# Sabre94/k8s-llm-monitor

Measured on AMD Instinct MI355X. Metric: diagnostic queries/sec (Llama-3-8B TP=1, /api/v1/query), higher is better.
Workload: dtype bf16; 1 GPU; model=llama-3-8b, global_batch=64, seq_len=2263, max_model_len=8192, parallelism=tp1, mode=wave, client=process, weight_layout=one (fragment-packed)

## Files before the change

k8s_llm_monitor_amd/ops/__init__.py:

```python
from __future__ import annotations

import importlib
import math
from collections import OrderedDict
from typing import Optional

import torch

from . import cpu_attn
from . import reference as ref

_EXT = None
_EXT_ERR: Optional[BaseException] = None


def native():
    global _EXT, _EXT_ERR
    if _EXT is None and _EXT_ERR is None:
        try:
            _EXT = importlib.import_module("k8s_llm_monitor_amd.ops._k8sllm_ops")
        except BaseException as e:
            _EXT_ERR = e
    if _EXT is None:
        raise RuntimeError(
# ... 438 lines not shown
    F2, K = w13.shape
    F = F2 // 2
    if F % 8:
        raise ValueError("interleave_gate_up8: F must be a multiple of 8")
    return w13.reshape(2, F // 8, 8, K).permute(1, 0, 2, 3).reshape(F2, K)


def deinterleave_gate_up8(w: torch.Tensor) -> torch.Tensor:
    F2, K = w.shape
    return w.reshape(F2 // 16, 2, 8, K).permute(1, 0, 2, 3).reshape(F2, K)


DEC_TABLE: dict = {
    (6144, 4096, 0): (4, 1, 6, 8),
    (4096, 4096, 0): (8, 1, 8, 8),
    (28672, 4096, 2): (1, 1, 7, 8),
    (4096, 14336, 0): (8, 1, 8, 8),
    (128256, 4096, 1): (1, 4, 8, 4),
    (151936, 4096, 1): (1, 2, 8, 8),
}

DEC_TABLE_M128: dict = {
    (6144, 4096, 0): (4, 1, 6, 8),
    (4096, 4096, 0): (8, 1, 8, 8),
    (28672, 4096, 2): (1, 1, 7, 8),
    (4096, 14336, 0): (8, 1, 8, 8),
    (128256, 4096, 1): (1, 2, 8, 8),
}


DEC_TABLE_F8: dict = {}

DEC_TABLE_F4: dict = {}


def dec_config(N: int, K: int, epi: int, experts: int = 1, rows: int = 0, f8: bool = False,
               f4: bool = False) -> Optional[tuple]:
    if (f8 or f4) and experts != 1:
        return None
    return _dec_pick(N, K, epi, experts, rows, f8, f4)


def _dec_pick(N: int, K: int, epi: int, experts: int, rows: int, f8: bool, f4: bool) -> Optional[tuple]:
    wide = rows > DEC_NARROW_MAX_M
    if wide and (experts != 1 or rows > DEC_MAX_M):
        return None
    if f8 and K % 64:
        return None
    if f4 and (f8 or K % 128):
        return None
    compiled = ([DEC_FORMS[i] for i in DEC_F8_FORMS] if f8 else
                [DEC_FORMS[i] for i, _ in DEC_F4_FORMS] if f4 else DEC_FORMS)
    if f8 and experts == 1 and (N, K, epi, 128 if wide else 64) in DEC_TABLE_F8:
        return DEC_TABLE_F8[(N, K, epi, 128 if wide else 64)]
    if f4 and experts == 1 and (N, K, epi, 128 if wide else 64) in DEC_TABLE_F4:
        return DEC_TABLE_F4[(N, K, epi, 128 if wide else 64)]
    hit = (DEC_TABLE_M128 if wide else DEC_TABLE).get((N, K, epi)) if experts == 1 else None
    if hit is not None and (not f8 or dec_form_ok(epi, hit, rows, f8=True)) and (
            not f4 or dec_form_ok(epi, hit, rows, f4=True, K=K)):
        return hit
    ntiles, ksteps = N // 16, K // 32
    forms = [f[1:4] for f in compiled
             if f[0] == epi and rows <= 16 * f[4] and f[:4] not in DEC_FORMS_TABLE_ONLY]
    cands = [(s,) + f for s in ((1, 2, 4, 8, 16) if epi == DEC_SLAB else (1,)) for f in forms]
    best = None
    for s, ntw, w, d in cands:
# ... 90 lines not shown
        for e in range(max(E, 1)):
            x = _cpu_a(a[e] if a.dim() == 5 else a, rows).float()
            wf = _cpu_w(w[e], wscale[e] if enc else None) if E else _cpu_w(w, wscale)
            if epi == 0:
                kc = K // S
                slabs = workspace[e * S * M * N: (e + 1) * S * M * N].view(S, M, N)
                for s in range(S):
                    y = x[:, s * kc:(s + 1) * kc] @ wf[:, s * kc:(s + 1) * kc].t()
                    slabs[s] = y * sc if sc is not None else y
                if row_w is not None:
                    slabs.mul_(row_w[:M, e].float().view(1, M, 1))
                continue
            y = x @ wf.t()
            if sc is not None:
                y = y * sc
            o = out[e] if E else out
            if epi == 1:
                o[:M].copy_(y.to(o.dtype))
            else:
                gu = deinterleave_gate_up8(y.to(a.dtype).float().t()).t()
                g, u = gu[:, : N // 2], gu[:, N // 2:]
                o.copy_(pack_activation((torch.nn.functional.silu(g) * u).to(a.dtype)))
        return max(E, 1) * S if epi == 0 else 1
    rn = (None, 0.0) if rownorm is None else (rownorm[0], float(rownorm[1]))
    wn = rownorm is not None and rownorm[0].shape[1] > 16
    ok = (dec_grouped_q_form_ok(epi, cfg, M, K=K, **enc_kw(w)) if E and enc else
          dec_form_ok(epi, cfg, M, grouped=E > 0, wide_norm=wn, f8=f8, f4=f4, K=K))
    if not ok:
        raise RuntimeError(f"{name}: form (epi, ntw, waves, depth) = {(epi,) + tuple(cfg[1:])} not compiled for "
                           f"{M} rows" + (" of a grouped launch" if E else "") +
                           (" with the wide deferred norm" if wn else "") +
                           (" over fp8 weights" if f8 else f" over mxfp4 weights in {S} K slices" if f4 else ""))
    r = native().gemm_dec(a, w, wscale if enc else None, workspace, out, S, epi, ntw, waves, depth, M, *rn,
                          row_w if E else None, DEC_F4_DEPTH_FORCE if f4 else 0)
    if r < 0:
        raise RuntimeError(f"{name}: configuration {cfg} not compiled for N={N} K={K} epi={epi}")
    return r


def dec_gemm(a: torch.Tensor, wp: torch.Tensor, epi: int, rows: int, workspace: Optional[torch.Tensor] = None,
             out: Optional[torch.Tensor] = None, rownorm: Optional[tuple] = None,
             cfg: Optional[tuple] = None, wscale: Optional[torch.Tensor] = None) -> int:
    return _dec_gemm("gemm_dec", a, wp, wscale, epi, rows, workspace, out, rownorm, None, cfg, 0)


def dec_gemm_grouped(a: torch.Tensor, wp: torch.Tensor, epi: int, rows: int, workspace: Optional[torch.Tensor] = None,
                     out: Optional[torch.Tensor] = None, row_w: Optional[torch.Tensor] = None,
                     cfg: Optional[tuple] = None) -> int:
    if wp.dtype == torch.uint8:
        raise ValueError("gemm_dec_grouped: grouped launches have no mxfp4 form here (dec_gemm_grouped_q takes the "
                         "codes with their scales)")
    return _dec_gemm("gemm_dec_grouped", a, wp, None, epi, rows, workspace, out, None, row_w, cfg, wp.shape[0])


def dec_gemm_grouped_q(a: torch.Tensor, wq: torch.Tensor, wqs: torch.Tensor, epi: int, rows: int,
                       workspace: Optional[torch.Tensor] = None, out: Optional[torch.Tensor] = None,
                       row_w: Optional[torch.Tensor] = None, cfg: Optional[tuple] = None) -> int:
    E = grouped_q_wdims(wq)[0]
    return _dec_gemm("gemm_dec_grouped_q", a, wq, wqs, epi, rows, workspace, out, None, row_w, cfg, E)


def dec_gemm_rc(a: torch.Tensor, wp: torch.Tensor, rows: int, residual: torch.Tensor, norm_w: torch.Tensor,
                eps: float) -> Optional[tuple]:
    N, K = skinny_wdims(wp)
    M = rows
    if K % 256 or N % 32 or M > 64:
        return None
# ... 929 lines not shown
```

k8s_llm_monitor_amd/ops/csrc/bindings.cpp:

```cpp
#include <torch/extension.h>
#include <c10/hip/HIPStream.h>
#include <hip/hip_runtime.h>

#include <cmath>

#include "gemm_dec_forms.h"
#include "gemm_skinny_plan.h"
#include "gemm_tile_forms.h"
#include "paged_decode_forms.h"

extern "C" {
int k8sllm_rmsnorm(void* out, const void* x, void* residual, const void* w, long rows, int d, float eps,
                   long x_stride, long out_stride, hipStream_t s);
int k8sllm_layernorm(void* out, const void* x, const void* w, const void* b, long rows, int d, float eps,
                     hipStream_t s);
int k8sllm_silu_mul(void* out, const void* x, long rows, int F, int interleaved, hipStream_t s);
int k8sllm_gelu_tanh(void* out, const void* x, long n, hipStream_t s);
int k8sllm_embedding(void* out, const int* ids, const void* weight, long T, int d, int vocab_start, int rows,
                     hipStream_t s);
int k8sllm_resolve_ids(int* out, const int* ids, const int* src, const int* prev, int n, hipStream_t s);
int k8sllm_rope_cache(void* qkv, long qkv_stride, const int* positions, const float* cos_sin, void* k_cache,
                      void* v_cache, const int* slot_mapping, long T, int Hq, int Hkv, int D, int block_size,
                      int apply_rope, const float* partial, int S, float* kv_scale, const void* q_norm_w,
                      const void* k_norm_w, float eps, int norm_bf16, hipStream_t s);
// ... 22 lines not shown
                            int nrows, const int* tok_off, const void* blob, int V, const int* eos_ids, int n_eos,
                            hipStream_t s);
int k8sllm_penalty_reset(void* table, long tstride, int V, int nslots, int slot, const int* ids, int n_prompt,
                         int n_out, float* pparams, float rep, float inv_rep, float presence, float frequency,
                         hipStream_t s);
int k8sllm_sample_parts(long B, int V);
long k8sllm_token_logprobs_ws(long B, int V);
int k8sllm_token_logprobs(int* out, const void* logits, int is_fp32, long B, long stride, int V, const int* tok,
                          const int* want, void* ws, hipStream_t s);
int k8sllm_moe_route(const void* logits, long T, int E, int K, int renorm, int* topk_ids, float* topk_w,
                     hipStream_t s);
int k8sllm_moe_router(const void* x, const void* wr, long T, int d, int E, int K, int renorm, int* ids, float* w,
                      float* wd, hipStream_t s);
int k8sllm_moe_align(const int* topk_ids, long n, int E, int* expert_offsets, int* sorted_idx, int* inv_idx,
                     hipStream_t s);
int k8sllm_moe_combine(void* out, const void* expert_out, const int* inv_idx, const float* topk_w, long T, int K,
                       int d, hipStream_t s);
int k8sllm_gather_rows(void* out, const void* x, const int* idx, long n, int d, int div, hipStream_t s);
int k8sllm_gemm_tile(const void* X, const void* W, void* Y, int M, int N, int K, const int* offsets, int E, long w_es,
                     int epi, int algo, const int* rope_pos, const float* rope_cs, int rope_heads,
                     const float* rs_part, int rs_np, float rs_eps, void* resid, void* hw, const void* norm_w,
                     float* ss_out, int wpk, const void* wscale, int wfmt, int persist, int cus, hipStream_t s);
int k8sllm_gemm_tile_forms(int* out, int cap);
int k8sllm_gemm_tile_persist_forms(int* out, int cap);
int k8sllm_moe_grouped_gemm(const void* X, const void* W, void* Y, const int* offsets, int E, long rows, int N, int K,
                            long w_es, int epi, hipStream_t s);
int k8sllm_gemm_skinny(const void* A, long lda, const void* Wp, float* partial, void* Y, long ldy, int M, int N, int K,
                       int S, int epi, int nt_tiles, int a_packed, const float* rn_ss, int rn_nc, int rn_d,
                       float rn_eps, int waves, int experts, long w_es, long a_es, long y_es,
                       const float* row_w, int row_w_ld, int w_rm, hipStream_t s);
int k8sllm_gemm_dec(const void* A, const void* W, const void* wscale, int wf, float* partial, void* Y, long ldy, int M,
                    int N, int K, int splits, int epi, int ntw, int waves, int depth, int f4_depth, const float* rn_ss,
                    int rn_nc, int rn_d, float rn_eps, int experts, long a_es, long w_eb, long s_eb, long y_es,
                    const float* rw, int rw_ld, hipStream_t s);
int k8sllm_gemm_dec_forms(int* out, int cap);
int k8sllm_gemm_dec_f8_forms(int* out, int cap);
int k8sllm_gemm_dec_f4_forms(int* out, int cap);
int k8sllm_gemm_dec_rc(const void* A, const void* Wp, void* resid, const void* nw, void* xw, float* ss, int M, int N,
                       int K, hipStream_t s);
int k8sllm_add_norm_partial(void* out, long out_stride, void* residual, const float* partial, int S, int M,
                            const void* w, int d, float* ss_part, hipStream_t s);
int k8sllm_embed_norm_partial(void* out, long out_stride, void* residual, const int* ids, const int* src,
                              const int* prev, const void* emb, int vocab, const void* w, int M, int d,
                              float* ss_part, hipStream_t s);
int k8sllm_reduce_slabs(void* out, const float* partial, int S, long n, hipStream_t s);
int k8sllm_reduce_add_rmsnorm(void* out, void* residual, const float* partial, int S, int M, const void* w, int d,
                              float eps, long out_stride, void* out2, hipStream_t s);
void* k8sllm_car_create(int rank, int world, long max_elems, void* handles, int* err);
int k8sllm_car_handle_size();
int k8sllm_car_open(void* state, const void* all_handles);
int k8sllm_car_all_reduce(void* state, const void* in, void* out, long n, long spin_limit, int algo, hipStream_t s);
int k8sllm_car_fused_tail(void* state, const float* slabs, int ns, long slab_stride, void* residual, const void* w,
                          void* out, long ldo, int M, int d, float eps, int packed, long spin_limit, int algo,
                          hipStream_t s);
int k8sllm_car_error(void* state);
int k8sllm_car_all_gather(void* state, const void* in, void* out, long n, long spin_limit, hipStream_t s);
int k8sllm_car_all_to_all(void* state, const void* in, void* out, long n, long spin_limit, hipStream_t s);
int k8sllm_car_error_async(void* state, void* host_dst, hipStream_t s);
void k8sllm_car_destroy(void* state);
}

namespace {

hipStream_t cur() { return c10::hip::getCurrentHIPStream().stream(); }

void check(int rc, const char* what) { TORCH_CHECK(rc == 0, "k8sllm kernel launch failed: ", what, " rc=", rc); }

// ... 677 lines not shown
  } else {
    TORCH_CHECK(a.dim() == 2 && a.stride(1) == 1 && a.stride(0) % 8 == 0, "gemm_skinny: a layout");
    TORCH_CHECK(a.size(1) == K, "gemm_skinny: a has ", a.size(1), " columns, weight K=", K);
    M = (int)a.size(0);
  }
  const int S = epi == 0 ? (int)splits : 1;
  const auto p = k8sllm::skinny_plan(M, N, K, S, (int)epi, (int)nt_tiles, a_packed ? 1 : 0, (int)waves, 1, w_rm);
  TORCH_CHECK(p.err == 0, "gemm_skinny: at most ", k8sllm::kSkinnyMaxM, " rows of a shape it tiles, rc=", p.err);
  float* pp = nullptr;
  void* yp = nullptr;
  long ldy = 0;
  if (epi == 0) {
    pp = slab_buffer(partial, (int64_t)p.slabs * M * N, "gemm_skinny");
  } else if (epi == 3) {
    yp = swiglu_packed_out(y, 0, M, N, "gemm_skinny");
  } else {
    TORCH_CHECK(y.has_value(), "gemm_skinny: output tensor required");
    dev_bf16(*y, "y");
    const int ncol = epi == 2 ? N / 2 : N;
    TORCH_CHECK(y->dim() == 2 && y->size(0) >= M && y->size(1) == ncol && y->stride(1) == 1, "gemm_skinny: y shape");
    ldy = y->stride(0);
    yp = y->data_ptr();
  }
  const float* rp = nullptr;
  int rn_nc = 0;
  rownorm_args(rn_ss, M, K, rp, rn_nc);
  check(k8sllm_gemm_skinny(a.data_ptr(), a_packed ? 0 : a.stride(0), wp.data_ptr(), pp, yp, ldy, M, N, K, S, (int)epi,
                           (int)nt_tiles, a_packed ? 1 : 0, rp, rn_nc, K, (float)rn_eps, (int)waves, 1, 0, 0, 0,
                           nullptr, 0, w_rm, cur()),
        "gemm_skinny");
  return p.slabs;
}

int64_t gemm_dec(torch::Tensor a, torch::Tensor w, c10::optional<torch::Tensor> wscale,
                 c10::optional<torch::Tensor> partial, c10::optional<torch::Tensor> y, int64_t splits, int64_t epi,
                 int64_t ntw, int64_t waves, int64_t depth, int64_t rows, c10::optional<torch::Tensor> rn_ss,
                 double rn_eps, c10::optional<torch::Tensor> row_w, int64_t f4_depth) {
  dev_bf16(a, "a");
  const auto wt = w.scalar_type();
  const int wf = wt == torch::kFloat8_e4m3fn ? k8sllm::DEC_W_F8 : wt == torch::kUInt8 ? k8sllm::DEC_W_F4 : k8sllm::DEC_W_BF16;
  const int g = w.dim() == 5 ? 1 : 0;
  const int kq = wf == k8sllm::DEC_W_F4 ? 128 : wf == k8sllm::DEC_W_F8 ? 64 : 32, wl = wf == k8sllm::DEC_W_BF16 ? 8 : 16;
  const std::string whats = std::string("gemm_dec (") + (wf == k8sllm::DEC_W_F4 ? "mxfp4" : wf == k8sllm::DEC_W_F8 ? "fp8" : "bf16") +
                            (g ? ", grouped)" : ")");
  const char* what = whats.c_str();
  TORCH_CHECK(w.is_cuda() && (wf != k8sllm::DEC_W_BF16 || wt == torch::kBFloat16) && w.dim() == 4 + g &&
                  w.is_contiguous() && w.size(g + 2) == 64 && w.size(g + 3) == wl,
              what, ": w must be bf16 [N/16, K/32, 64, 8], float8_e4m3fn [N/16, K/64, 64, 16] or uint8 [N/16, K/128, "
                    "64, 16], fragment-packed, or an [E, ...] stack of such");
  const int E = g ? (int)w.size(0) : 0, N = (int)w.size(g) * 16, K = (int)w.size(g + 1) * kq, M = (int)rows;
  const void* sp = nullptr;
  if (wf == k8sllm::DEC_W_F8) {
    TORCH_CHECK(wscale.has_value() && wscale->is_cuda() && wscale->scalar_type() == torch::kFloat32 &&
                    wscale->is_contiguous() && (g ? wscale->dim() == 2 && wscale->size(0) == E && wscale->size(1) == N
                                                  : wscale->numel() == N),
                what, ": wscale must be [N] fp32 ([E, N] for a stack)");
    sp = wscale->data_ptr();
  } else if (wf == k8sllm::DEC_W_F4) {
    TORCH_CHECK(wscale.has_value() && wscale->is_cuda() && wscale->scalar_type() == torch::kUInt8 &&
                    wscale->is_contiguous() && wscale->dim() == 4 + g && (!g || wscale->size(0) == E) &&
                    wscale->size(g) == w.size(g) && wscale->size(g + 1) == w.size(g + 1) &&
                    wscale->size(g + 2) == 16 && wscale->size(g + 3) == 4,
                what, ": wscale must be uint8 [N/16, K/128, 16, 4] ([E, ...] for a stack)");
    sp = wscale->data_ptr();
  }
  TORCH_CHECK(g || !row_w.has_value(), what, ": routing weights go with an [E, ...] stack");
  TORCH_CHECK(!g || !rn_ss.has_value(), what, ": a grouped launch takes no deferred norm");
  TORCH_CHECK(!g || epi == 0 || epi == 2, what, ": only the slab and SwiGLU outputs");
  const float* rp = nullptr;
  int rn_nc = 0;
  rownorm_args(rn_ss, M, K, rp, rn_nc);
  const bool scaled = epi == 0 && row_w.has_value();
  const k8sllm::DecPlan p = k8sllm::dec_plan(wf, M, N, K, (int)splits, (int)epi, (int)ntw, (int)waves, (int)depth,
                                             (int)f4_depth, E, scaled, rn_nc);
  const int MT = (M + 15) / 16;
  TORCH_CHECK(M > 0 && M <= p.max_m && (!g || E >= 1), what, ": 1..", p.max_m, " rows", g ? ", >= 1 expert" : "");
  const bool per_e = g && a.dim() == 5;
  const int ag = per_e ? 1 : 0;
  TORCH_CHECK(a.is_contiguous() && a.dim() == 4 + ag && (!per_e || a.size(0) == E) && a.size(ag) >= MT &&
                  a.size(ag + 1) * 32 == K && a.size(ag + 2) == 64 && a.size(ag + 3) == 8,
              what, ": a must be fragment-packed [ceil(M/16), K/32, 64, 8]", g ? " or [E, ...]" : "");
  if (p.err < 0) return -1;
  float* pp = nullptr;
  void* yp = nullptr;
  long ldy = 0, y_es = 0;
  const float* rw = nullptr;
  int rw_ld = 0;
  if (epi == 0) {
    pp = slab_buffer(partial, (int64_t)p.slabs * M * N, what);
    if (scaled) {
      TORCH_CHECK(row_w->is_cuda() && row_w->scalar_type() == torch::kFloat32 && row_w->dim() == 2 &&
                      row_w->size(0) >= M && row_w->size(1) == E && row_w->stride(1) == 1,
                  what, ": row_w [M, E] fp32");
      rw = row_w->data_ptr<float>();
      rw_ld = (int)row_w->stride(0);
    }
  } else if (epi == 2) {
    yp = swiglu_packed_out(y, E, M, N, what);
    y_es = g ? y->stride(0) : 0;
  } else {
    TORCH_CHECK(y.has_value(), what, ": output tensor required");
    dev_bf16(*y, "y");
    TORCH_CHECK(y->dim() == 2 && y->size(0) >= M && y->size(1) == N && y->stride(1) == 1, what, ": y [M, N]");
    ldy = y->stride(0);
    yp = y->data_ptr();
  }
  const long a_es = per_e ? a.stride(0) : 0, w_eb = g ? w.stride(0) * w.element_size() : 0;
  const long s_eb = g && sp ? wscale->stride(0) * wscale->element_size() : 0;
  const int rc = k8sllm_gemm_dec(a.data_ptr(), w.data_ptr(), sp, wf, pp, yp, ldy, M, N, K, (int)splits, (int)epi,
                                 (int)ntw, (int)waves, (int)depth, (int)f4_depth, rp, rn_nc, K, (float)rn_eps, E,
                                 a_es, w_eb, s_eb, y_es, rw, rw_ld, cur());
  if (rc < 0) return -1;
  check(rc, what);
  return p.slabs;
}

std::vector<int64_t> gemm_dec_plan(int64_t wf, int64_t M, int64_t N, int64_t K, int64_t splits, int64_t epi, int64_t ntw,
                                   int64_t waves, int64_t depth, int64_t f4_depth, int64_t experts, bool has_row_w,
                                   int64_t rn_nc) {
  const k8sllm::DecPlan p = k8sllm::dec_plan((int)wf, (int)M, (int)N, (int)K, (int)splits, (int)epi, (int)ntw,
                                             (int)waves, (int)depth, (int)f4_depth, (int)experts, has_row_w, (int)rn_nc);
  return {p.err, p.mt, p.kchunk, p.d4, p.rnw, p.gx, p.gy, p.gz, p.slabs, p.max_m};
}

std::vector<int64_t> gemm_dec_f8_forms() {
  std::vector<int> v(k8sllm::kDecNF8Forms);
  const int n = k8sllm_gemm_dec_f8_forms(v.data(), k8sllm::kDecNF8Forms);
  TORCH_CHECK(n == k8sllm::kDecNF8Forms, "gemm_dec_f8_forms: ", n, " rows compiled, ", k8sllm::kDecNF8Forms,
              " in the header");
  return std::vector<int64_t>(v.begin(), v.end());
}

std::vector<std::vector<int64_t>> gemm_dec_f4_forms() {
  std::vector<int> v(2 * k8sllm::kDecNF4Forms);
  const int n = k8sllm_gemm_dec_f4_forms(v.data(), k8sllm::kDecNF4Forms);
  TORCH_CHECK(n == k8sllm::kDecNF4Forms, "gemm_dec_f4_forms: ", n, " rows compiled, ", k8sllm::kDecNF4Forms,
              " in the header");
  std::vector<std::vector<int64_t>> out;
  for (int i = 0; i < n; ++i) out.push_back({v[2 * i], v[2 * i + 1]});
  return out;
}

std::vector<std::tuple<int64_t, int64_t, int64_t, int64_t, int64_t, int64_t>> gemm_dec_forms() {
  std::vector<int> v(6 * k8sllm::kDecNForms);
  const int n = k8sllm_gemm_dec_forms(v.data(), k8sllm::kDecNForms);
  TORCH_CHECK(n == k8sllm::kDecNForms, "gemm_dec_forms: ", n, " rows compiled, ", k8sllm::kDecNForms,
              " in the header");
  std::vector<std::tuple<int64_t, int64_t, int64_t, int64_t, int64_t, int64_t>> rows;
  for (int i = 0; i < n; ++i)
    rows.emplace_back(v[6 * i], v[6 * i + 1], v[6 * i + 2], v[6 * i + 3], v[6 * i + 4], v[6 * i + 5]);
  return rows;
}

std::vector<std::vector<int64_t>> gemm_skinny_forms() {
  std::vector<std::vector<int64_t>> rows;
// ... 257 lines not shown
        py::arg("cus") = (int64_t)k8sllm::kTileCUs, py::arg("ext") = false);
  m.def("gemm_tile_forms", &gemm_tile_forms);
  m.def("gemm_tile_persist_forms", &gemm_tile_persist_forms);
  m.def("gelu_tanh", &gelu_tanh);
  m.def("embedding", &embedding);
  m.def("resolve_ids", &resolve_ids);
  m.def("rope_and_cache", &rope_and_cache);
  m.def("paged_decode", &paged_decode);
  m.def("paged_decode_fused", &paged_decode_fused);
  m.def("paged_decode_plan", &paged_decode_plan);
  m.def("paged_decode_forms", &paged_decode_forms);
  m.def("decode_tw_force", [](int64_t tw) { k8sllm_decode_tw_force((int)tw); });
  m.def("flash_prefill", &flash_prefill);
  m.def("embed_norm_partial", &embed_norm_partial);
  m.def("sample", &sample, py::arg("out"), py::arg("logits"), py::arg("temps"), py::arg("top_k"), py::arg("top_p"),
        py::arg("rng"), py::arg("advance") = false, py::arg("pen_table") = py::none(),
        py::arg("pen_params") = py::none(), py::arg("pen_slots") = py::none(), py::arg("pen_vocab") = 0,
        py::arg("g_mask") = py::none(), py::arg("g_trans") = py::none(), py::arg("g_state") = py::none(),
        py::arg("g_slots") = py::none(), py::arg("g_tok_off") = py::none(), py::arg("g_blob") = py::none(),
        py::arg("g_eos") = py::none());
  m.def("guide_mask_build", &guide_mask_build);
  m.def("penalty_reset", &penalty_reset);
  m.def("token_logprobs", &token_logprobs);
  m.def("moe_route", &moe_route);
  m.def("moe_router", &moe_router);
  m.def("moe_align", &moe_align);
  m.def("moe_combine", &moe_combine);
  m.def("gather_rows", &gather_rows);
  m.def("gemm_skinny", &gemm_skinny);
  m.def("gemm_skinny_grouped", &gemm_skinny_grouped);
  m.def("gemm_skinny_forms", &gemm_skinny_forms);
  m.def("gemm_skinny_plan", &gemm_skinny_plan);
  m.def("gemm_dec_plan", &gemm_dec_plan);
  m.attr("SKINNY_MAX_M") = k8sllm::kSkinnyMaxM;
  m.attr("SKINNY_GROUPED_MAX_M") = k8sllm::kSkinnyGroupedMaxM;
  m.def("gemm_dec", &gemm_dec);
  m.def("gemm_dec_forms", &gemm_dec_forms);
  m.def("gemm_dec_f8_forms", &gemm_dec_f8_forms);
  m.def("gemm_dec_f4_forms", &gemm_dec_f4_forms);
  m.def("gemm_dec_rc", &gemm_dec_rc);
  m.def("reduce_add_rms_norm", &reduce_add_rms_norm);
  m.def("reduce_slabs", &reduce_slabs);
  m.def("add_norm_partial", &add_norm_partial);
  m.def("car_create", &car_create);
  m.def("car_open", &car_open);
  m.def("car_all_reduce", &car_all_reduce, py::arg("state"), py::arg("in"), py::arg("out"), py::arg("spin_limit"),
        py::arg("algo") = -1);
  m.def("car_fused_tail", &car_fused_tail);
  m.def("car_all_to_all", &car_all_to_all);
  m.def("car_error", &car_error);
  m.def("car_all_gather", &car_all_gather);
  m.def("car_error_async", &car_error_async);
  m.def("car_destroy", &car_destroy);
}
```

k8s_llm_monitor_amd/ops/csrc/gemm_dec_forms.h:

```cpp
#pragma once

namespace k8sllm {

enum { DEC_SLAB = 0, DEC_BF16 = 1, DEC_SWIGLU8 = 2 };
enum { DEC_W_BF16 = 0, DEC_W_F8 = 1, DEC_W_F4 = 2 };

struct DecForm {
  int epi, ntw, waves, depth, max_mt, wide_norm;
};

constexpr DecForm kDecForms[] = {
    {DEC_SLAB, 1, 8, 8, 8, 0},
    {DEC_SLAB, 1, 6, 8, 8, 0},
    {DEC_SLAB, 1, 4, 16, 4, 0},
    {DEC_SLAB, 1, 4, 8, 8, 0},
    {DEC_SWIGLU8, 1, 7, 8, 8, 1},
    {DEC_SWIGLU8, 1, 7, 16, 4, 1},
    {DEC_SWIGLU8, 1, 8, 16, 4, 0},
    {DEC_BF16, 4, 8, 4, 4, 0},
    {DEC_BF16, 3, 8, 8, 4, 0},
    {DEC_BF16, 2, 8, 8, 8, 0},
    {DEC_BF16, 1, 8, 8, 4, 0},
};
constexpr int kDecNForms = sizeof(kDecForms) / sizeof(kDecForms[0]);
// ... 12 lines not shown
};
constexpr DecF4Form kDecF4Forms[] = {{0, 16}, {1, 16}, {4, 16}, {7, 8}, {9, 16}};
constexpr int kDecNF4Forms = sizeof(kDecF4Forms) / sizeof(kDecF4Forms[0]);

constexpr int dec_form_f4_depth(int form) {
  for (const DecF4Form& f : kDecF4Forms)
    if (f.form == form) return f.depth;
  return 0;
}

constexpr int dec_max_mt() {
  int m = 0;
  for (const DecForm& f : kDecForms) m = f.max_mt > m ? f.max_mt : m;
  return m;
}

constexpr int kDecNarrowMaxMT = 4;
constexpr int kDecMaxM = 16 * dec_max_mt();
constexpr int kDecNarrowMaxM = 16 * kDecNarrowMaxMT;

constexpr int kDecAChunk = 8;
constexpr int kDecRnNarrow = 16;
constexpr int kDecRnWide = 256;

struct DecPlan {
  int err;
  int max_m;
  int mt;
  int kchunk;
  int d4;
  int rnw;
  int gx, gy, gz;
  int slabs;
};

constexpr int dec_form_index(int epi, int ntw, int waves, int depth) {
  for (int i = 0; i < kDecNForms; ++i) {
    const DecForm& f = kDecForms[i];
    if (f.epi == epi && f.ntw == ntw && f.waves == waves && f.depth == depth) return i;
  }
  return -1;
}

constexpr DecPlan dec_plan(int wf, int M, int N, int K, int splits, int epi, int ntw, int waves, int depth,
                           int f4_depth, int experts, bool has_row_w, int rn_nc) {
  DecPlan p{-1, 0, 0, 0, 0, 0, 0, 0, 0, 0};
  const bool grouped = experts >= 1 || has_row_w, quant = wf != DEC_W_BF16;
  p.max_m = grouped ? kDecNarrowMaxM : kDecMaxM;
  if ((wf != DEC_W_BF16 && wf != DEC_W_F8 && wf != DEC_W_F4) || experts < 0 || M < 1 || M > p.max_m) return p;
  if (has_row_w && epi != DEC_SLAB) return p;
  if (quant && grouped && ((epi != DEC_SLAB && epi != DEC_SWIGLU8) || rn_nc > 0)) return p;
  if (N % 16 || K % (wf == DEC_W_F4 ? 128 : wf == DEC_W_F8 ? 64 : 32) || splits < 1 || K % splits) return p;
  const int form = dec_form_index(epi, ntw, waves, depth);
  if (ntw * waves < 1 || (wf == DEC_W_F4 && (form < 0 || dec_form_f4_depth(form) == 0))) return p.err = -5, p;
  p.mt = (M + 15) / 16;
  p.kchunk = K / splits;
  const int ks = p.kchunk / 32;
  p.err = -3;
  if (wf == DEC_W_F4) {
    if (p.kchunk % 128 || ks < kDecAChunk || ks % kDecAChunk) return p;
    const int dmax = p.mt > 1 ? 8 : dec_form_f4_depth(form);
    p.d4 = f4_depth ? f4_depth : dmax >= 16 && ks % 16 == 0 ? 16 : 8;
    if ((p.d4 != 8 && p.d4 != 16) || p.d4 > dmax || ks % p.d4) return p;
  } else {
    const int iter = depth > kDecAChunk ? depth : kDecAChunk;
    if (p.kchunk % 32 || ks < iter || ks % iter) return p;
  }
  if (epi != DEC_SLAB && splits != 1) return p.err = -4, p;
  p.rnw = rn_nc > kDecRnNarrow;
  if (p.rnw && (quant || rn_nc % 16 || rn_nc > kDecRnWide)) return p.err = -1, p;
  int max_mt = 0;
  if (form >= 0) {
    const DecForm& f = kDecForms[form];
    if (wf == DEC_W_F8) max_mt = dec_form_f8(form) ? f.max_mt : 0;
    else if (wf == DEC_W_F4) max_mt = p.d4 == 16 ? 1 : f.max_mt;
    else max_mt = p.rnw ? (f.wide_norm ? kDecNarrowMaxMT : 0) : f.max_mt;
  }
  if (p.mt > max_mt) return p.err = -5, p;
  const int nwg = ntw * waves;
  p.gx = (N / 16 + nwg - 1) / nwg;
  p.gy = splits;
  p.gz = experts > 1 ? experts : 1;
  p.slabs = epi == DEC_SLAB ? p.gz * splits : 1;
  p.err = 0;
  return p;
}

}
```

k8s_llm_monitor_amd/ops/csrc/gemm_decode.hip:

```cpp
#include <type_traits>

#include "common.h"
#include "gemm_dec_forms.h"

namespace k8sllm {

typedef unsigned int u32x4 __attribute__((ext_vector_type(4)));

struct DecGroup {
  long a_es, y_es;
  long w_eb, s_eb;
  const float* rw;
  int rw_ld;
};

__device__ __forceinline__ __amdgpu_buffer_rsrc_t dec_rsrc(const void* base, long bytes) {
  const uint64_t a = reinterpret_cast<uint64_t>(base);
  const uint32_t lo = __builtin_amdgcn_readfirstlane((uint32_t)a), hi = __builtin_amdgcn_readfirstlane((uint32_t)(a >> 32));
  const int nb = __builtin_amdgcn_readfirstlane((int)min(bytes, 0x7fffffffL));
  return __builtin_amdgcn_make_buffer_rsrc(reinterpret_cast<void*>(((uint64_t)hi << 32) | lo), 0, nb, 0x00020000);
}
constexpr int kRnMax = 4;
constexpr int kRnWide = 16;

constexpr int kDecCH = 8;

template <int MT, int WAVES>
struct DecGeom {
  static constexpr int SLOT = kDecCH * MT * 1024;
  static constexpr int PIECES = kDecCH * MT * 64;
  static constexpr int NLD = (PIECES + 64 * WAVES - 1) / (64 * WAVES);
};

__device__ __forceinline__ bf16x8 dec_f8x8(uint32_t lo, uint32_t hi) {
  typedef __bf16 bf16x2 __attribute__((ext_vector_type(2)));
  const bf16x2 a = __builtin_amdgcn_cvt_scalef32_pk_bf16_fp8(lo, 1.0f, false);
  const bf16x2 b = __builtin_amdgcn_cvt_scalef32_pk_bf16_fp8(lo, 1.0f, true);
  const bf16x2 c = __builtin_amdgcn_cvt_scalef32_pk_bf16_fp8(hi, 1.0f, false);
  const bf16x2 d = __builtin_amdgcn_cvt_scalef32_pk_bf16_fp8(hi, 1.0f, true);
  return bf16x8{a[0], a[1], b[0], b[1], c[0], c[1], d[0], d[1]};
}

__device__ __forceinline__ bf16x8 dec_f4x8(uint32_t q, float scale) {
  typedef __bf16 bf16x2 __attribute__((ext_vector_type(2)));
  const bf16x2 a = __builtin_amdgcn_cvt_scalef32_pk_bf16_fp4(q, scale, 0);
  const bf16x2 b = __builtin_amdgcn_cvt_scalef32_pk_bf16_fp4(q, scale, 1);
  const bf16x2 c = __builtin_amdgcn_cvt_scalef32_pk_bf16_fp4(q, scale, 2);
  const bf16x2 d = __builtin_amdgcn_cvt_scalef32_pk_bf16_fp4(q, scale, 3);
  return bf16x8{a[0], a[1], b[0], b[1], c[0], c[1], d[0], d[1]};
}

template <int MT, int NTW, int WAVES, int EPI, int DEPTH, bool RNW = false, int WF = DEC_W_BF16>
__global__ __launch_bounds__(64 * WAVES, 1) void gemm_dec_kernel(
    const bf16_t* __restrict__ A, const bf16_t* __restrict__ W, float* __restrict__ partial,
    bf16_t* __restrict__ Y, long ldy, int M, int N, int K, int kchunk, const float* __restrict__ rn_ss, int rn_nc,
    float rn_inv_d, float rn_eps, DecGroup grp, const float* __restrict__ wscale) {
  constexpr bool F8 = WF == DEC_W_F8, F4 = WF == DEC_W_F4;
  static_assert(!F8 || (!RNW && DEPTH % 2 == 0), "fp8 weights: narrow deferred norm, whole k-step pairs in the ring");
  static_assert(!F4 || (!RNW && DEPTH % 4 == 0), "mxfp4 weights: narrow deferred norm, whole k-step quads in the ring");
  using G = DecGeom<MT, WAVES>;
  const int ex = blockIdx.z;
  A += ex * grp.a_es;
  W = reinterpret_cast<const bf16_t*>(reinterpret_cast<const char*>(W) + ex * grp.w_eb);
  if constexpr (F8 || F4) wscale = reinterpret_cast<const float*>(reinterpret_cast<const char*>(wscale) + ex * grp.s_eb);
  if constexpr (EPI == DEC_SWIGLU8) Y += ex * grp.y_es;
  constexpr int ITER = DEPTH > kDecCH ? DEPTH : kDecCH;
  __shared__ __attribute__((aligned(16))) char sA[2 * G::SLOT];
  __shared__ float s_inv[MT * 16];
  const int wave = __builtin_amdgcn_readfirstlane(threadIdx.x >> 6), lane = threadIdx.x & 63;
  const int ksteps = K >> 5;
  const int kb = blockIdx.y * (kchunk >> 5);
  const int nsteps = kchunk >> 5;
  const int niter = nsteps / ITER;
  const int tile0 = (blockIdx.x * WAVES + wave) * NTW;

  constexpr int WSH = F4 ? 2 : F8 ? 1 : 0;
  constexpr int RING = DEPTH >> WSH;
  const int wsteps = ksteps >> WSH, wkb = kb >> WSH;
  const u32x4* wp[NTW];
#pragma unroll
  for (int t = 0; t < NTW; ++t)
    wp[t] = reinterpret_cast<const u32x4*>(W) + ((long)min(tile0 + t, (N >> 4) - 1) * wsteps + wkb) * 64 + lane;
  float wsc[F8 ? NTW : 1];
  if constexpr (F8) {
#pragma unroll
    for (int t = 0; t < NTW; ++t) wsc[t] = wscale[min(tile0 + t, (N >> 4) - 1) * 16 + (lane & 15)];
  }
  const uint32_t* sp[F4 ? NTW : 1];
  if constexpr (F4) {
#pragma unroll
    for (int t = 0; t < NTW; ++t)
      sp[t] = reinterpret_cast<const uint32_t*>(wscale) + ((long)min(tile0 + t, (N >> 4) - 1) * wsteps + wkb) * 16 + (lane & 15);
  }
  u32x4 wr[RING][NTW];
  uint32_t wsr[F4 ? RING : 1][F4 ? NTW : 1];
  auto ring_fill = [&]() {
#pragma unroll
    for (int d = 0; d < RING; ++d)
#pragma unroll
      for (int t = 0; t < NTW; ++t) {
        wr[d][t] = __builtin_nontemporal_load(wp[t] + d * 64);
        if constexpr (F4) wsr[d][t] = __builtin_nontemporal_load(sp[t] + d * 16);
      }
  };

  constexpr int RNP = (MT * 64 + 64 * WAVES - 1) / (64 * WAVES);
  static_assert(!RNW || RNP == 1, "the wide deferred-norm form serves <= 64 rows (behind gemm_dec_rc)");
// ... 146 lines not shown
          const uint32_t e8 = (wsr[(j % DEPTH) >> 2][t] >> (8 * (j & 3))) & 0xffu;
          b = dec_f4x8(wr[(j % DEPTH) >> 2][t][j & 3], __uint_as_float(e8 << 23));
        } else {
          b = __builtin_bit_cast(bf16x8, wr[j % DEPTH][t]);
        }
#pragma unroll
        for (int m = 0; m < MT; ++m) acc[m][t] = __builtin_amdgcn_mfma_f32_16x16x32_bf16(af[m], b, acc[m][t], 0, 0, 0);
      }
      if constexpr (F8) {
        if ((j & 1) && (!LAST || j + DEPTH < ITER)) {
#pragma unroll
          for (int t = 0; t < NTW; ++t)
            wr[(j % DEPTH) >> 1][t] = __builtin_nontemporal_load(wp[t] + ((ks + DEPTH) >> 1) * 64);
        }
      } else if constexpr (F4) {
        if ((j & 3) == 3 && (!LAST || j + DEPTH < ITER)) {
#pragma unroll
          for (int t = 0; t < NTW; ++t) {
            wr[(j % DEPTH) >> 2][t] = __builtin_nontemporal_load(wp[t] + ((ks + DEPTH) >> 2) * 64);
            wsr[(j % DEPTH) >> 2][t] = __builtin_nontemporal_load(sp[t] + ((ks + DEPTH) >> 2) * 16);
          }
        }
      } else if (!LAST || j + DEPTH < ITER) {
#pragma unroll
        for (int t = 0; t < NTW; ++t) wr[j % DEPTH][t] = __builtin_nontemporal_load(wp[t] + (ks + DEPTH) * 64);
      }
      __builtin_amdgcn_sched_barrier(0);
    }
  };
  int it = 0;
  for (; it + 1 < niter; ++it) iteration(it, std::false_type{});
  iteration(it, std::true_type{});

#pragma unroll
  for (int m = 0; m < MT; ++m) {
    float rs[4];
#pragma unroll
    for (int r = 0; r < 4; ++r) rs[r] = rn_ss != nullptr ? s_inv[m * 16 + (lane >> 4) * 4 + r] : 1.f;
#pragma unroll
    for (int t = 0; t < NTW; ++t) {
      const int tile = tile0 + t;
      if (tile >= (N >> 4)) continue;
      if constexpr (EPI == DEC_SWIGLU8) {
        const int F = N >> 1;
        const int f = tile * 8 + (lane & 7);
#pragma unroll
        for (int r = 0; r < 4; ++r) {
          float v = acc[m][t][r] * rs[r];
          if constexpr (F8) v *= wsc[t];
          const float o = __shfl_xor(v, 8, kWave);
          const int row = m * 16 + (lane >> 4) * 4 + r;
          if ((lane & 8) == 0) {
            const float g = bf2f(f2bf(v)), u = bf2f(f2bf(o));
            Y[(((long)(row >> 4) * (F >> 5) + (f >> 5)) * 64 + ((f >> 3) & 3) * 16 + (row & 15)) * 8 + (f & 7)] =
                f2bf(g * u / (1.f + __expf(-g)));
          }
        }
      } else {
        const int col = tile * 16 + (lane & 15);
#pragma unroll
        for (int r = 0; r < 4; ++r) {
          const int row = m * 16 + (lane >> 4) * 4 + r;
          if (row < M) {
            float v = acc[m][t][r] * rs[r];
            if constexpr (F8) v *= wsc[t];
            if constexpr (EPI == DEC_BF16)
              Y[(long)row * ldy + col] = f2bf(v);
            else
              partial[((long)(ex * gridDim.y + blockIdx.y) * M + row) * N + col] =
                  grp.rw != nullptr ? v * grp.rw[(long)row * grp.rw_ld + ex] : v;
          }
        }
      }
    }
  }
}


template <int MT, int DEPTH, int NKS>
__global__ __launch_bounds__(512, 1) void gemm_dec_rc_kernel(const bf16_t* __restrict__ A, const bf16_t* __restrict__ W,
                                                             bf16_t* __restrict__ resid, const bf16_t* __restrict__ nw,
                                                             bf16_t* __restrict__ xw, float* __restrict__ ss_out,
                                                             int M, int N, int K) {
  constexpr int WAVES = 8;
  static_assert(NKS % DEPTH == 0, "the ring consumes whole DEPTH groups of k-steps");
  __shared__ __attribute__((aligned(16))) f32x4 red[WAVES][MT][64];
  const int wave = __builtin_amdgcn_readfirstlane(threadIdx.x >> 6), lane = threadIdx.x & 63;
  const int tile = blockIdx.x;
  const int ksteps = K >> 5;
  constexpr int nks = NKS;
  const int kb = wave * nks;
  const u32x4* wp = reinterpret_cast<const u32x4*>(W) + ((long)tile * ksteps + kb) * 64 + lane;
  const u32x4* ap[MT];
#pragma unroll
  for (int m = 0; m < MT; ++m) ap[m] = reinterpret_cast<const u32x4*>(A) + ((long)m * ksteps + kb) * 64 + lane;
  u32x4 rw[DEPTH], ra[DEPTH][MT];
#pragma unroll
  for (int d = 0; d < DEPTH; ++d) {
    rw[d] = __builtin_nontemporal_load(wp + d * 64);
#pragma unroll
    for (int m = 0; m < MT; ++m) ra[d][m] = ap[m][d * 64];
  }
// ... 40 lines not shown
      xw[act_index(row, col, -(long)(N >> 5))] = f2bf(hv * wcol);
    }
  }
#pragma unroll
  for (int r = 0; r < 4; ++r) {
    float v = ssr[r];
#pragma unroll
    for (int o = 1; o < 16; o <<= 1) v += __shfl_xor(v, o, kWave);
    const int row = m * 16 + (lane >> 4) * 4 + r;
    if ((lane & 15) == 0 && row < M) ss_out[(long)row * (N >> 4) + tile] = v;
  }
}

}

using namespace k8sllm;

namespace {

struct DecLaunch {
  dim3 grid, blk;
  hipStream_t s;
  const bf16_t *A, *W;
  float* partial;
  bf16_t* Y;
  long ldy;
  int M, N, K, kchunk;
  const float* rn_ss;
  int rn_nc;
  float inv_d, rn_eps;
  DecGroup dg;
  const float* wscale;
  int d4 = 0;
};

template <int F, bool RNW, int MT, int WF = DEC_W_BF16, int D4 = 0>
bool dec_launch(int mt, const DecLaunch& l) {
  if constexpr (MT == 0) {
    return false;
  } else {
    if (mt != MT) return dec_launch<F, RNW, MT - 1, WF, D4>(mt, l);
    constexpr DecForm f = kDecForms[F];
    constexpr int depth = WF == DEC_W_F4 ? D4 : f.depth;
    hipLaunchKernelGGL((gemm_dec_kernel<MT, f.ntw, f.waves, f.epi, depth, RNW, WF>), l.grid, l.blk, 0, l.s, l.A,
                       l.W, l.partial, l.Y, l.ldy, l.M, l.N, l.K, l.kchunk, l.rn_ss, l.rn_nc, l.inv_d, l.rn_eps, l.dg,
                       l.wscale);
    return true;
  }
}

template <int WF = DEC_W_BF16, int F = 0>
bool dec_dispatch(int epi, int ntw, int waves, int depth, bool rnw, int mt, const DecLaunch& l) {
  if constexpr (F == kDecNForms) {
    return false;
  } else {
    constexpr DecForm f = kDecForms[F];
    if (epi != f.epi || ntw != f.ntw || waves != f.waves || depth != f.depth)
      return dec_dispatch<WF, F + 1>(epi, ntw, waves, depth, rnw, mt, l);
    if constexpr (WF == DEC_W_F8)
      return !rnw && dec_launch<F, false, dec_form_f8(F) ? f.max_mt : 0, DEC_W_F8>(mt, l);
    else if constexpr (WF == DEC_W_F4) {
      constexpr int d1 = dec_form_f4_depth(F);
      if (rnw) return false;
      if (l.d4 == 16) return dec_launch<F, false, d1 >= 16 ? 1 : 0, DEC_W_F4, 16>(mt, l);
      return l.d4 == 8 && dec_launch<F, false, d1 >= 8 ? f.max_mt : 0, DEC_W_F4, 8>(mt, l);
    }
    else
      return rnw ? dec_launch<F, true, f.wide_norm ? kDecNarrowMaxMT : 0>(mt, l) : dec_launch<F, false, f.max_mt>(mt, l);
  }
}

}

static_assert(kDecAChunk == kDecCH && kDecRnNarrow == 4 * kRnMax && kDecRnWide == 16 * kRnWide,
              "dec_plan (gemm_dec_forms.h) plans with the kernel's constants");

extern "C" int k8sllm_gemm_dec(const void* A, const void* W, const void* wscale, int wf, float* partial, void* Y,
                               long ldy, int M, int N, int K, int splits, int epi, int ntw, int waves, int depth,
                               int f4_depth, const float* rn_ss, int rn_nc, int rn_d, float rn_eps, int experts,
                               long a_es, long w_eb, long s_eb, long y_es, const float* rw, int rw_ld,
                               hipStream_t s) {
  if (M <= 0) return 0;
  if (wf != DEC_W_BF16 && wscale == nullptr) return -1;
  const DecPlan p = dec_plan(wf, M, N, K, splits, epi, ntw, waves, depth, f4_depth, experts, rw != nullptr,
                             rn_ss != nullptr ? rn_nc : 0);
  if (p.err < 0) return p.err;
  const DecLaunch l{dim3(p.gx, p.gy, p.gz), dim3(64 * waves), s, (const bf16_t*)A, (const bf16_t*)W, partial,
                    (bf16_t*)Y, ldy, M, N, K, p.kchunk, rn_ss, rn_nc, rn_d > 0 ? 1.f / (float)rn_d : 0.f, rn_eps,
                    DecGroup{a_es, y_es, w_eb, s_eb, rw, rw_ld}, wf == DEC_W_BF16 ? nullptr : (const float*)wscale,
                    p.d4};
  bool ok = false;
  switch (wf) {
    case DEC_W_BF16: ok = dec_dispatch<DEC_W_BF16>(epi, ntw, waves, depth, p.rnw, p.mt, l); break;
    case DEC_W_F8: ok = dec_dispatch<DEC_W_F8>(epi, ntw, waves, depth, false, p.mt, l); break;
    case DEC_W_F4: ok = dec_dispatch<DEC_W_F4>(epi, ntw, waves, depth, false, p.mt, l); break;
  }
  if (!ok) return -5;
  return (int)hipGetLastError();
}

extern "C" int k8sllm_gemm_dec_f8_forms(int* out, int cap) {
  for (int i = 0; i < kDecNF8Forms && i < cap; ++i) out[i] = kDecF8Forms[i];
  return kDecNF8Forms;
}

extern "C" int k8sllm_gemm_dec_f4_forms(int* out, int cap) {
  for (int i = 0; i < kDecNF4Forms && i < cap; ++i) {
    out[2 * i] = kDecF4Forms[i].form;
    out[2 * i + 1] = kDecF4Forms[i].depth;
  }
  return kDecNF4Forms;
}

extern "C" int k8sllm_gemm_dec_forms(int* out, int cap) {
  for (int i = 0; i < kDecNForms && i < cap; ++i) {
    const DecForm& f = kDecForms[i];
    const int row[6] = {f.epi, f.ntw, f.waves, f.depth, f.max_mt, f.wide_norm};
    for (int j = 0; j < 6; ++j) out[6 * i + j] = row[j];
  }
  return kDecNForms;
}


// ... 24 lines not shown
```

Before: 25.24 queries/s.

## Stage split-K slab partials through LDS for coalesced row stores and XCD-aware block mapping

In the split-K slab epilogue of the decode GEMM, the fp32 accumulators are first staged into the now-unused A ring in shared memory. They are then written back as full 128-bit rows through buffer stores, optionally with a cache-policy bit, instead of scattered per-lane scalar stores. A second change remaps workgroup IDs so that the split slices of one column tile land on the same XCD, aiming for better L2 locality during the reduction. Both are on by default for more than 16 rows (XCD remap always), which adds an extra LDS round trip and barriers per tile and relies on correct alignment and size guards.

Measured after the change: 25.62 queries/s, median of 6. 1.5% higher.

```diff
diff --git a/k8s_llm_monitor_amd/ops/__init__.py b/k8s_llm_monitor_amd/ops/__init__.py
--- a/k8s_llm_monitor_amd/ops/__init__.py
+++ b/k8s_llm_monitor_amd/ops/__init__.py
@@ -494,6 +494,36 @@
 DEC_TABLE_F8: dict = {}
 
 DEC_TABLE_F4: dict = {}
+
+
+DEC_SLAB_ROWS = -1
+DEC_SLAB_WT = -1
+DEC_XCD_SPLITS = -1
+
+
+def dec_slab_shipped(rows: int) -> tuple:
+    wide = int(rows > 16)
+    return (wide, wide, 1)
+
+
+def dec_xcd_ok(gx: int, splits: int) -> bool:
+    return splits in (2, 4, 8) and (gx * splits) % 8 == 0
+
+
+def dec_xcd_map(L: int, splits: int) -> tuple:
+    c, j, per = L % 8, L // 8, 8 // splits
+    return j * per + c // splits, c % splits
+
+
+def dec_slab_plan(M: int, N: int, cfg: tuple, grouped: bool = False, sw: Optional[tuple] = None) -> tuple:
+    sr, sw_, sx = (DEC_SLAB_ROWS, DEC_SLAB_WT, DEC_XCD_SPLITS) if sw is None else sw
+    S, ntw, waves, _ = cfg
+    d = dec_slab_shipped(M)
+    gx = -(-(N // 16) // (ntw * waves))
+    rows = int((d[0] if sr < 0 else sr) != 0 and M > 16 and M * N * 4 < 0x7fffffff)
+    wt = int(bool(rows) and (d[1] if sw_ < 0 else sw_) != 0)
+    xcd = int((d[2] if sx < 0 else sx) != 0 and not grouped and dec_xcd_ok(gx, S))
+    return rows, wt, xcd
 
 
 def dec_config(N: int, K: int, epi: int, experts: int = 1, rows: int = 0, f8: bool = False,
@@ -650,7 +680,8 @@
                            (" with the wide deferred norm" if wn else "") +
                            (" over fp8 weights" if f8 else f" over mxfp4 weights in {S} K slices" if f4 else ""))
     r = native().gemm_dec(a, w, wscale if enc else None, workspace, out, S, epi, ntw, waves, depth, M, *rn,
-                          row_w if E else None, DEC_F4_DEPTH_FORCE if f4 else 0)
+                          row_w if E else None, DEC_F4_DEPTH_FORCE if f4 else 0, DEC_SLAB_ROWS, DEC_SLAB_WT,
+                          DEC_XCD_SPLITS)
     if r < 0:
         raise RuntimeError(f"{name}: configuration {cfg} not compiled for N={N} K={K} epi={epi}")
     return r
diff --git a/k8s_llm_monitor_amd/ops/csrc/bindings.cpp b/k8s_llm_monitor_amd/ops/csrc/bindings.cpp
--- a/k8s_llm_monitor_amd/ops/csrc/bindings.cpp
+++ b/k8s_llm_monitor_amd/ops/csrc/bindings.cpp
@@ -78,7 +78,7 @@
 int k8sllm_gemm_dec(const void* A, const void* W, const void* wscale, int wf, float* partial, void* Y, long ldy, int M,
                     int N, int K, int splits, int epi, int ntw, int waves, int depth, int f4_depth, const float* rn_ss,
                     int rn_nc, int rn_d, float rn_eps, int experts, long a_es, long w_eb, long s_eb, long y_es,
-                    const float* rw, int rw_ld, hipStream_t s);
+                    const float* rw, int rw_ld, int sw_rows, int sw_wt, int sw_xcd, hipStream_t s);
 int k8sllm_gemm_dec_forms(int* out, int cap);
 int k8sllm_gemm_dec_f8_forms(int* out, int cap);
 int k8sllm_gemm_dec_f4_forms(int* out, int cap);
@@ -822,10 +822,11 @@
   return p.slabs;
 }
 
-int64_t gemm_dec(torch::Tensor a, torch::Tensor w, c10::optional<torch::Tensor> wscale,
-                 c10::optional<torch::Tensor> partial, c10::optional<torch::Tensor> y, int64_t splits, int64_t epi,
-                 int64_t ntw, int64_t waves, int64_t depth, int64_t rows, c10::optional<torch::Tensor> rn_ss,
-                 double rn_eps, c10::optional<torch::Tensor> row_w, int64_t f4_depth) {
+int64_t gemm_dec_sw(torch::Tensor a, torch::Tensor w, c10::optional<torch::Tensor> wscale,
+                    c10::optional<torch::Tensor> partial, c10::optional<torch::Tensor> y, int64_t splits, int64_t epi,
+                    int64_t ntw, int64_t waves, int64_t depth, int64_t rows, c10::optional<torch::Tensor> rn_ss,
+                    double rn_eps, c10::optional<torch::Tensor> row_w, int64_t f4_depth, int64_t sw_rows,
+                    int64_t sw_wt, int64_t sw_xcd) {
   dev_bf16(a, "a");
   const auto wt = w.scalar_type();
   const int wf = wt == torch::kFloat8_e4m3fn ? k8sllm::DEC_W_F8 : wt == torch::kUInt8 ? k8sllm::DEC_W_F4 : k8sllm::DEC_W_BF16;
@@ -862,7 +863,7 @@
   rownorm_args(rn_ss, M, K, rp, rn_nc);
   const bool scaled = epi == 0 && row_w.has_value();
   const k8sllm::DecPlan p = k8sllm::dec_plan(wf, M, N, K, (int)splits, (int)epi, (int)ntw, (int)waves, (int)depth,
-                                             (int)f4_depth, E, scaled, rn_nc);
+                                             (int)f4_depth, E, scaled, rn_nc, (int)sw_rows, (int)sw_wt, (int)sw_xcd);
   const int MT = (M + 15) / 16;
   TORCH_CHECK(M > 0 && M <= p.max_m && (!g || E >= 1), what, ": 1..", p.max_m, " rows", g ? ", >= 1 expert" : "");
   const bool per_e = g && a.dim() == 5;
@@ -899,18 +900,33 @@
   const long s_eb = g && sp ? wscale->stride(0) * wscale->element_size() : 0;
   const int rc = k8sllm_gemm_dec(a.data_ptr(), w.data_ptr(), sp, wf, pp, yp, ldy, M, N, K, (int)splits, (int)epi,
                                  (int)ntw, (int)waves, (int)depth, (int)f4_depth, rp, rn_nc, K, (float)rn_eps, E,
-                                 a_es, w_eb, s_eb, y_es, rw, rw_ld, cur());
+                                 a_es, w_eb, s_eb, y_es, rw, rw_ld, (int)sw_rows, (int)sw_wt, (int)sw_xcd, cur());
   if (rc < 0) return -1;
   check(rc, what);
   return p.slabs;
 }
 
+int64_t gemm_dec(torch::Tensor a, torch::Tensor w, c10::optional<torch::Tensor> wscale,
+                 c10::optional<torch::Tensor> partial, c10::optional<torch::Tensor> y, int64_t splits, int64_t epi,
+                 int64_t ntw, int64_t waves, int64_t depth, int64_t rows, c10::optional<torch::Tensor> rn_ss,
+                 double rn_eps, c10::optional<torch::Tensor> row_w, int64_t f4_depth) {
+  return gemm_dec_sw(a, w, wscale, partial, y, splits, epi, ntw, waves, depth, rows, rn_ss, rn_eps, row_w, f4_depth,
+                     -1, -1, -1);
+}
+
+std::vector<int64_t> gemm_dec_plan_sw(int64_t wf, int64_t M, int64_t N, int64_t K, int64_t splits, int64_t epi,
+                                      int64_t ntw, int64_t waves, int64_t depth, int64_t f4_depth, int64_t experts,
+                                      bool has_row_w, int64_t rn_nc, int64_t sw_rows, int64_t sw_wt, int64_t sw_xcd) {
+  const k8sllm::DecPlan p = k8sllm::dec_plan((int)wf, (int)M, (int)N, (int)K, (int)splits, (int)epi, (int)ntw,
+                                             (int)waves, (int)depth, (int)f4_depth, (int)experts, has_row_w, (int)rn_nc,
+                                             (int)sw_rows, (int)sw_wt, (int)sw_xcd);
+  return {p.err, p.mt, p.kchunk, p.d4, p.rnw, p.gx, p.gy, p.gz, p.slabs, p.max_m, p.rows, p.wt, p.xcd};
+}
+
 std::vector<int64_t> gemm_dec_plan(int64_t wf, int64_t M, int64_t N, int64_t K, int64_t splits, int64_t epi, int64_t ntw,
                                    int64_t waves, int64_t depth, int64_t f4_depth, int64_t experts, bool has_row_w,
                                    int64_t rn_nc) {
-  const k8sllm::DecPlan p = k8sllm::dec_plan((int)wf, (int)M, (int)N, (int)K, (int)splits, (int)epi, (int)ntw,
-                                             (int)waves, (int)depth, (int)f4_depth, (int)experts, has_row_w, (int)rn_nc);
-  return {p.err, p.mt, p.kchunk, p.d4, p.rnw, p.gx, p.gy, p.gz, p.slabs, p.max_m};
+  return gemm_dec_plan_sw(wf, M, N, K, splits, epi, ntw, waves, depth, f4_depth, experts, has_row_w, rn_nc, -1, -1, -1);
 }
 
 std::vector<int64_t> gemm_dec_f8_forms() {
@@ -1234,9 +1250,11 @@
   m.def("gemm_skinny_forms", &gemm_skinny_forms);
   m.def("gemm_skinny_plan", &gemm_skinny_plan);
   m.def("gemm_dec_plan", &gemm_dec_plan);
+  m.def("gemm_dec_plan", &gemm_dec_plan_sw);
   m.attr("SKINNY_MAX_M") = k8sllm::kSkinnyMaxM;
   m.attr("SKINNY_GROUPED_MAX_M") = k8sllm::kSkinnyGroupedMaxM;
   m.def("gemm_dec", &gemm_dec);
+  m.def("gemm_dec", &gemm_dec_sw);
   m.def("gemm_dec_forms", &gemm_dec_forms);
   m.def("gemm_dec_f8_forms", &gemm_dec_f8_forms);
   m.def("gemm_dec_f4_forms", &gemm_dec_f4_forms);
diff --git a/k8s_llm_monitor_amd/ops/csrc/gemm_dec_forms.h b/k8s_llm_monitor_amd/ops/csrc/gemm_dec_forms.h
--- a/k8s_llm_monitor_amd/ops/csrc/gemm_dec_forms.h
+++ b/k8s_llm_monitor_amd/ops/csrc/gemm_dec_forms.h
@@ -68,7 +68,23 @@
   int rnw;
   int gx, gy, gz;
   int slabs;
+  int rows;
+  int wt;
+  int xcd;
 };
+
+enum { kDecRows = 1, kDecWt = 2, kDecXcd = 4 };
+
+struct DecXY {
+  int x, y;
+};
+constexpr bool dec_xcd_ok(int gx, int splits) {
+  return (splits == 2 || splits == 4 || splits == 8) && (gx * splits) % 8 == 0;
+}
+constexpr DecXY dec_xcd_map(int L, int splits) {
+  const int c = L & 7, j = L >> 3, per = 8 / splits;
+  return DecXY{j * per + c / splits, c % splits};
+}
 
 constexpr int dec_form_index(int epi, int ntw, int waves, int depth) {
   for (int i = 0; i < kDecNForms; ++i) {
@@ -78,9 +94,18 @@
   return -1;
 }
 
+struct DecSlabSw {
+  int rows, wt, xcd;
+};
+constexpr DecSlabSw dec_slab_shipped(int M) {
+  const int wide = M > 16;
+  return DecSlabSw{wide, wide, 1};
+}
+
 constexpr DecPlan dec_plan(int wf, int M, int N, int K, int splits, int epi, int ntw, int waves, int depth,
-                           int f4_depth, int experts, bool has_row_w, int rn_nc) {
-  DecPlan p{-1, 0, 0, 0, 0, 0, 0, 0, 0, 0};
+                           int f4_depth, int experts, bool has_row_w, int rn_nc, int sw_rows = -1, int sw_wt = -1,
+                           int sw_xcd = -1) {
+  DecPlan p{-1, 0, 0, 0, 0, 0, 0, 0, 0, 0, 0, 0, 0};
   const bool grouped = experts >= 1 || has_row_w, quant = wf != DEC_W_BF16;
   p.max_m = grouped ? kDecNarrowMaxM : kDecMaxM;
   if ((wf != DEC_W_BF16 && wf != DEC_W_F8 && wf != DEC_W_F4) || experts < 0 || M < 1 || M > p.max_m) return p;
@@ -118,6 +143,12 @@
   p.gy = splits;
   p.gz = experts > 1 ? experts : 1;
   p.slabs = epi == DEC_SLAB ? p.gz * splits : 1;
+  if (epi == DEC_SLAB) {
+    const DecSlabSw d = dec_slab_shipped(M);
+    p.rows = (sw_rows < 0 ? d.rows : sw_rows) != 0 && p.mt > 1 && (long)M * N * 4 < 0x7fffffffL;
+    p.wt = p.rows && (sw_wt < 0 ? d.wt : sw_wt) != 0;
+    p.xcd = (sw_xcd < 0 ? d.xcd : sw_xcd) != 0 && !grouped && dec_xcd_ok(p.gx, splits);
+  }
   p.err = 0;
   return p;
 }
diff --git a/k8s_llm_monitor_amd/ops/csrc/gemm_decode.hip b/k8s_llm_monitor_amd/ops/csrc/gemm_decode.hip
--- a/k8s_llm_monitor_amd/ops/csrc/gemm_decode.hip
+++ b/k8s_llm_monitor_amd/ops/csrc/gemm_decode.hip
@@ -24,6 +24,7 @@
 constexpr int kRnWide = 16;
 
 constexpr int kDecCH = 8;
+constexpr int kDecSC1 = 16;
 
 template <int MT, int WAVES>
 struct DecGeom {
@@ -54,7 +55,7 @@
 __global__ __launch_bounds__(64 * WAVES, 1) void gemm_dec_kernel(
     const bf16_t* __restrict__ A, const bf16_t* __restrict__ W, float* __restrict__ partial,
     bf16_t* __restrict__ Y, long ldy, int M, int N, int K, int kchunk, const float* __restrict__ rn_ss, int rn_nc,
-    float rn_inv_d, float rn_eps, DecGroup grp, const float* __restrict__ wscale) {
+    float rn_inv_d, float rn_eps, DecGroup grp, const float* __restrict__ wscale, int flags) {
   constexpr bool F8 = WF == DEC_W_F8, F4 = WF == DEC_W_F4;
   static_assert(!F8 || (!RNW && DEPTH % 2 == 0), "fp8 weights: narrow deferred norm, whole k-step pairs in the ring");
   static_assert(!F4 || (!RNW && DEPTH % 4 == 0), "mxfp4 weights: narrow deferred norm, whole k-step quads in the ring");
@@ -69,10 +70,18 @@
   __shared__ float s_inv[MT * 16];
   const int wave = __builtin_amdgcn_readfirstlane(threadIdx.x >> 6), lane = threadIdx.x & 63;
   const int ksteps = K >> 5;
-  const int kb = blockIdx.y * (kchunk >> 5);
+  int bx = blockIdx.x, by = blockIdx.y;
+  if constexpr (EPI == DEC_SLAB) {
+    if (flags & kDecXcd) {
+      const DecXY m = dec_xcd_map(blockIdx.x + gridDim.x * blockIdx.y, gridDim.y);
+      bx = m.x;
+      by = m.y;
+    }
+  }
+  const int kb = by * (kchunk >> 5);
   const int nsteps = kchunk >> 5;
   const int niter = nsteps / ITER;
-  const int tile0 = (blockIdx.x * WAVES + wave) * NTW;
+  const int tile0 = (bx * WAVES + wave) * NTW;
 
   constexpr int WSH = F4 ? 2 : F8 ? 1 : 0;
   constexpr int RING = DEPTH >> WSH;
@@ -285,6 +294,44 @@
   for (; it + 1 < niter; ++it) iteration(it, std::false_type{});
   iteration(it, std::true_type{});
 
+  if constexpr (EPI == DEC_SLAB && MT > 1) {
+    if (flags & kDecRows) {
+      constexpr int COLS = 16 * NTW * WAVES, LD = COLS + 4, PPR = COLS / 4;
+      static_assert(MT * 16 * LD * 4 <= 2 * G::SLOT, "the row image fits the dead A ring");
+      static_assert((MT * 16 * PPR) % (64 * WAVES) == 0, "whole passes of the workgroup over the image");
+      float* img = reinterpret_cast<float*>(sA);
+      __syncthreads();
+#pragma unroll
+      for (int m = 0; m < MT; ++m)
+#pragma unroll
+        for (int t = 0; t < NTW; ++t)
+#pragma unroll
+          for (int r = 0; r < 4; ++r) {
+            const int rl = m * 16 + (lane >> 4) * 4 + r;
+            float v = acc[m][t][r] * (rn_ss != nullptr ? s_inv[rl] : 1.f);
+            if constexpr (F8) v *= wsc[t];
+            if (grp.rw != nullptr && rl < M) v = v * grp.rw[(long)rl * grp.rw_ld + ex];
+            img[rl * LD + (wave * NTW + t) * 16 + (lane & 15)] = v;
+          }
+      __syncthreads();
+      const __amdgpu_buffer_rsrc_t rs = dec_rsrc(partial + (long)(ex * gridDim.y + by) * M * N, (long)M * N * 4);
+      const int col0 = bx * COLS;
+#pragma unroll
+      for (int q0 = 0; q0 < MT * 16 * PPR; q0 += 64 * WAVES) {
+        const int q = q0 + threadIdx.x;
+        const int row = q / PPR, c = (q % PPR) * 4;
+        if (row < M && col0 + c < N) {
+          const u32x4 v = *reinterpret_cast<const u32x4*>(img + row * LD + c);
+          const uint32_t off = (uint32_t)((row * N + col0 + c) * 4);
+          if (flags & kDecWt)
+            __builtin_amdgcn_raw_buffer_store_b128(v, rs, off, 0, kDecSC1);
+          else
+            __builtin_amdgcn_raw_buffer_store_b128(v, rs, off, 0, 0);
+        }
+      }
+      return;
+    }
+  }
 #pragma unroll
   for (int m = 0; m < MT; ++m) {
     float rs[4];
@@ -320,7 +367,7 @@
             if constexpr (EPI == DEC_BF16)
               Y[(long)row * ldy + col] = f2bf(v);
             else
-              partial[((long)(ex * gridDim.y + blockIdx.y) * M + row) * N + col] =
+              partial[((long)(ex * gridDim.y + by) * M + row) * N + col] =
                   grp.rw != nullptr ? v * grp.rw[(long)row * grp.rw_ld + ex] : v;
           }
         }
@@ -427,6 +474,7 @@
   DecGroup dg;
   const float* wscale;
   int d4 = 0;
+  int flags = 0;
 };
 
 template <int F, bool RNW, int MT, int WF = DEC_W_BF16, int D4 = 0>
@@ -439,7 +487,7 @@
     constexpr int depth = WF == DEC_W_F4 ? D4 : f.depth;
     hipLaunchKernelGGL((gemm_dec_kernel<MT, f.ntw, f.waves, f.epi, depth, RNW, WF>), l.grid, l.blk, 0, l.s, l.A,
                        l.W, l.partial, l.Y, l.ldy, l.M, l.N, l.K, l.kchunk, l.rn_ss, l.rn_nc, l.inv_d, l.rn_eps, l.dg,
-                       l.wscale);
+                       l.wscale, l.flags);
     return true;
   }
 }
@@ -474,16 +522,18 @@
                                long ldy, int M, int N, int K, int splits, int epi, int ntw, int waves, int depth,
                                int f4_depth, const float* rn_ss, int rn_nc, int rn_d, float rn_eps, int experts,
                                long a_es, long w_eb, long s_eb, long y_es, const float* rw, int rw_ld,
-                               hipStream_t s) {
+                               int sw_rows, int sw_wt, int sw_xcd, hipStream_t s) {
   if (M <= 0) return 0;
   if (wf != DEC_W_BF16 && wscale == nullptr) return -1;
   const DecPlan p = dec_plan(wf, M, N, K, splits, epi, ntw, waves, depth, f4_depth, experts, rw != nullptr,
-                             rn_ss != nullptr ? rn_nc : 0);
+                             rn_ss != nullptr ? rn_nc : 0, sw_rows, sw_wt, sw_xcd);
   if (p.err < 0) return p.err;
+  const bool rows = p.rows && reinterpret_cast<uintptr_t>(partial) % 16 == 0;
+  const int flags = (rows ? kDecRows : 0) | (rows && p.wt ? kDecWt : 0) | (p.xcd ? kDecXcd : 0);
   const DecLaunch l{dim3(p.gx, p.gy, p.gz), dim3(64 * waves), s, (const bf16_t*)A, (const bf16_t*)W, partial,
                     (bf16_t*)Y, ldy, M, N, K, p.kchunk, rn_ss, rn_nc, rn_d > 0 ? 1.f / (float)rn_d : 0.f, rn_eps,
                     DecGroup{a_es, y_es, w_eb, s_eb, rw, rw_ld}, wf == DEC_W_BF16 ? nullptr : (const float*)wscale,
-                    p.d4};
+                    p.d4, flags};
   bool ok = false;
   switch (wf) {
     case DEC_W_BF16: ok = dec_dispatch<DEC_W_BF16>(epi, ntw, waves, depth, p.rnw, p.mt, l); break;
```
